# rrahn/libspm

Measured on AMD Instinct MI355X. Metric: Gbases/s scanned, Myers k<=3 |P|=100, higher is better.
Workload: dtype u32

## Files before the change

libspm_amd/csrc/filter.hpp:

```cpp
#pragma once

#include "brute.hpp"
#include "common.hpp"
#include "filter_shared.hpp"
#include "pack.hpp"
#include "hd.hpp"

namespace spm_hip
{

struct survivor
{
    uint32_t key;
    uint32_t t_lo, t_hi;
    uint32_t pad;
};
constexpr uint32_t kSurvInvalid = 0xFFFFFFFFu;

struct band_rec
{
    uint32_t slot;
    uint32_t val;
    uint32_t seg;
    uint32_t band;
};
constexpr uint32_t kBandInvalid = 0xFFFFFFFFu;
constexpr unsigned long long kBandEmpty = ~0ull;

constexpr uint32_t kChunkMax = 1024;
constexpr uint32_t kCandLdsSlot = 4;
constexpr uint32_t kCandRec = 8;

struct filter_params
{
    const uint8_t *text;
    uint64_t text_alloc;
    uint64_t lo, hi;
    uint32_t stride;
    uint32_t bitmap_words;
    uint32_t n_probes;
    uint32_t span_chunks;
    uint32_t span_unit;
    uint32_t dynamic;
    uint32_t key_len;
    uint32_t key_mask;
    uint32_t hash_variant;
    uint32_t lds_words;
    uint32_t chd_slot_mask;
    uint32_t chd_bucket_shift;
    uint32_t chd_disp_off;
    const uint32_t *bitmap;
    uint32_t span_budget;
    uint32_t pass;
    uint32_t anchor_c, anchor_cm;
    uint32_t n_pat, pat_c[kDensePatterns], pat_cm[kDensePatterns];
    uint32_t bucket_shift;
    const uint4 *buckets;
    survivor *surv;
    unsigned long long *counters;
    uint64_t surv_cap;
    uint64_t *ovf_spans;
    uint64_t ovf_cap;
};

__device__ __forceinline__ void wave_count_add(unsigned long long *counter, uint32_t v)
{
    for (int o = 32; o > 0; o >>= 1)
        v += __shfl_xor(v, o);
    if ((threadIdx.x & 63) == 0 && v)
        atomicAdd(counter, (unsigned long long)v);
}

__device__ __forceinline__ uint32_t *cand_chunk_of(const filter_params &P, const uint32_t *lds)
{
    const uint32_t wave = (uint32_t)__builtin_amdgcn_readfirstlane(threadIdx.x >> 6);
    return const_cast<uint32_t *>(lds) + P.lds_words + kCandLdsSlot + kCandRec * wave;
}

__device__ __forceinline__ void span_open(const filter_params &P, const uint32_t *lds, uint32_t lane, uint64_t begin)
{
    if (lane == 0) {
        uint32_t *ck = cand_chunk_of(P, lds);
        ck[4] = 0;
        ck[5] = 0;
        ck[6] = (uint32_t)begin;
        ck[7] = (uint32_t)(begin >> 32);
    }
}

__device__ __forceinline__ void span_give_up(const filter_params &P, uint32_t *ck, uint32_t lane)
{
    if (lane == 0) {
        ck[5] = 1;
        const unsigned long long i = atomicAdd(&P.counters[kCntSpansGaveUp], 1ull);
        if (i < P.ovf_cap) {
            P.ovf_spans[2 * i] = ((uint64_t)ck[7] << 32) | ck[6];
            P.ovf_spans[2 * i + 1] = (uint64_t)P.span_chunks * (uint64_t)P.span_unit;
        } else {
            atomicAdd(&P.counters[kCntVoid], 1ull);
        }
    }
    __builtin_amdgcn_fence(__ATOMIC_RELEASE, "wavefront");
    __builtin_amdgcn_wave_barrier();
}

__device__ __forceinline__ void surv_close(const filter_params &P, const uint32_t *ck, uint32_t lane)
{
    const uint32_t used = ck[2], size = ck[3];
    const uint64_t base = ((uint64_t)ck[1] << 32) | ck[0];
    for (uint32_t i = used + lane; i < size; i += 64)
        if (base + i < P.surv_cap) {
            survivor sv;
            sv.key = 0;
            sv.t_lo = 0;
            sv.t_hi = kSurvInvalid;
            sv.pad = 0;
            P.surv[base + i] = sv;
        }
}

__device__ __forceinline__ void emit_survivors(const filter_params &P, bool has, uint32_t key, uint64_t t, uint32_t lane,
                                               const uint32_t *lds)
{
    const uint64_t m = __ballot(has);
    if (m == 0)
        return;
    uint32_t *ck = cand_chunk_of(P, lds);
    const uint32_t n = __popcll(m);
    uint32_t used = (uint32_t)__builtin_amdgcn_readfirstlane(ck[2]);
    const uint32_t size = (uint32_t)__builtin_amdgcn_readfirstlane(ck[3]);
    const uint32_t cnt = (uint32_t)__builtin_amdgcn_readfirstlane(ck[4]) + n;
    if (cnt > P.span_budget) {
        span_give_up(P, ck, lane);
        return;
    }
    if (used + n > size) {
        surv_close(P, ck, lane);
        uint32_t next = size * 2 < kChunkMin ? kChunkMin : (size * 2 > kChunkMax ? kChunkMax : size * 2);
        next = next < n ? n : next;
        if (lane == 0) {
            const unsigned long long b = atomicAdd(&P.counters[kCntSurvSlots], (unsigned long long)next);
            ck[0] = (uint32_t)b;
            ck[1] = (uint32_t)(b >> 32);
            ck[2] = 0;
            ck[3] = next;
        }
        used = 0;
        __builtin_amdgcn_fence(__ATOMIC_RELEASE, "wavefront");
        __builtin_amdgcn_wave_barrier();
    }
    const uint64_t cbase = ((uint64_t)(uint32_t)__builtin_amdgcn_readfirstlane(ck[1]) << 32) |
                           (uint32_t)__builtin_amdgcn_readfirstlane(ck[0]);
    if (cbase + used + n > P.surv_cap) {
        span_give_up(P, ck, lane);
        return;
    }
    if (has) {
        survivor sv;
        sv.key = key;
        sv.t_lo = (uint32_t)t;
        sv.t_hi = (uint32_t)(t >> 32);
        sv.pad = P.pass;
        P.surv[cbase + used + __popcll(m & ((1ull << lane) - 1))] = sv;
    }
    if (lane == 0) {
        ck[2] = used + n;
        ck[4] = cnt;
    }
    __builtin_amdgcn_fence(__ATOMIC_RELEASE, "wavefront");
    __builtin_amdgcn_wave_barrier();
}

template <int S, int NWD, int HV, int SIG, bool PK, bool KM>
__device__ __forceinline__ void filter_words(const filter_params &P, const uint32_t (&w)[NWD],
                                             const uint32_t (&prev)[NWD], const uint32_t (&nv)[SIG != 4 ? NWD : 1],
                                             uint64_t gbase, uint32_t lane, const uint32_t *lds, uint32_t idx_mask)
{
    constexpr int NWIN = 16 / S;
    const uint32_t kmask = KM ? P.key_mask : 0xFFFFFFFFu;
    static_assert(NWD * NWIN <= 32, "one mask bit per window of a group");
    uint32_t pos_mask = 0;
    if constexpr (HV == 2) {
        const uint16_t *fp_tab = reinterpret_cast<const uint16_t *>(lds);
        const uint16_t *disp_tab = reinterpret_cast<const uint16_t *>(reinterpret_cast<const uint8_t *>(lds) + P.chd_disp_off);
        uint32_t xs[NWD * NWIN], ds[NWD * NWIN];
#pragma unroll
        for (int u = 0; u < NWD; ++u) {
#pragma unroll
            for (int i = 0; i < NWIN; ++i) {
                const int d = S * (i + 1);
                const uint32_t key = (d == 16 ? w[u] : alignbit(w[u], prev[u], (2 * d) & 31)) & kmask;
                const uint32_t x = chd_hash(key).x;
                xs[u * NWIN + i] = x;
                ds[u * NWIN + i] = disp_tab[x >> P.chd_bucket_shift];
            }
        }
#pragma unroll
        for (int u = 0; u < NWD; ++u) {
#pragma unroll
            for (int i = 0; i < NWIN; ++i) {
                const int d = S * (i + 1);
                const uint32_t key = (d == 16 ? w[u] : alignbit(w[u], prev[u], (2 * d) & 31)) & kmask;
                const uint32_t slot = ((xs[u * NWIN + i] >> 3) + ds[u * NWIN + i] * ((key | 1u) & 0xFFFFFFu)) &
                                      P.chd_slot_mask;
                ds[u * NWIN + i] = fp_tab[slot];
            }
        }
#pragma unroll
        for (int u = 0; u < NWD; ++u) {
#pragma unroll
            for (int i = 0; i < NWIN; ++i) {
                const int d = S * (i + 1);
                const uint32_t key = (d == 16 ? w[u] : alignbit(w[u], prev[u], (2 * d) & 31)) & kmask;
                const uint32_t miss = (ds[u * NWIN + i] ^ key ^ (key >> 16)) & 0xFFFFu;
                pos_mask |= (miss == 0 ? 1u : 0u) << (u * NWIN + i);
            }
        }
    } else {
#pragma unroll
        for (int u = 0; u < NWD; ++u) {
#pragma unroll
            for (int i = 0; i < NWIN; ++i) {
                const int d = S * (i + 1);
                const uint32_t key = (d == 16 ? w[u] : alignbit(w[u], prev[u], (2 * d) & 31)) & kmask;
                const uint32_t h = bloom_hash(key, 0) & idx_mask;
                const uint32_t word = lds[h >> 5];
                pos_mask |= __builtin_amdgcn_ubfe(word, h, 1) << (u * NWIN + i);
            }
        }
        for (uint32_t pr = 1; pr < P.n_probes; ++pr) {
            if (__ballot(pos_mask != 0) == 0)
                break;
            uint32_t keep = 0;
#pragma unroll
            for (int u = 0; u < NWD; ++u) {
#pragma unroll
                for (int i = 0; i < NWIN; ++i) {
                    if (pos_mask & (1u << (u * NWIN + i))) {
                        const int d = S * (i + 1);
                        const uint32_t key = (d == 16 ? w[u] : alignbit(w[u], prev[u], (2 * d) & 31)) & kmask;
                        const uint32_t h = bloom_hash(key, pr) & idx_mask;
                        const uint32_t word = lds[h >> 5];
                        keep |= __builtin_amdgcn_ubfe(word, h, 1) << (u * NWIN + i);
                    }
                }
            }
            pos_mask = keep;
        }
    }
    if constexpr (SIG != 4) {
        if (__ballot(pos_mask != 0) != 0) {
#pragma unroll
            for (int u = 0; u < NWD; ++u) {
#pragma unroll
                for (int i = 0; i < NWIN; ++i) {
                    const int d = S * (i + 1);
                    if (__builtin_amdgcn_ubfe(nv[u], d, P.key_len) != 0)
                        pos_mask &= ~(1u << (u * NWIN + i));
                }
            }
        }
    }
    while (__ballot(pos_mask != 0) != 0) {
        if (__builtin_amdgcn_readfirstlane(cand_chunk_of(P, lds)[5]) != 0)
            break;
        uint64_t t = 0;
        uint32_t key = 0;
        bool has = false;
        if (pos_mask != 0) {
            const int bit = __ffs(pos_mask) - 1;
            pos_mask &= pos_mask - 1;
            const int u = bit / NWIN, i = bit % NWIN;
            const int d = S * (i + 1);
            uint32_t wu = w[0], pu = prev[0];
#pragma unroll
            for (int q = 1; q < NWD; ++q)
                if (u == q) {
                    wu = w[q];
                    pu = prev[q];
                }
            key = (d == 16 ? wu : alignbit(wu, pu, (uint32_t)(2 * d) & 31u)) & kmask;
            const uint64_t wpos = PK ? gbase + (uint64_t)(u >> 2) * 4096 + (uint64_t)lane * 64 + (uint64_t)(u & 3) * 16
                                     : gbase + (uint64_t)u * 1024 + (uint64_t)lane * 16;
            const int64_t ts = (int64_t)wpos - 16 + d;
            if (ts >= (int64_t)P.lo && (uint64_t)ts + P.key_len <= P.hi) {
                t = (uint64_t)ts;
                has = true;
            }
        }
        emit_survivors(P, has, key, t, lane, lds);
    }
}



__device__ __forceinline__ uint32_t anchor_select(uint32_t w, uint32_t prev, uint32_t c, uint32_t cm)
{
    const uint32_t C0 = (c & 3u) * 0x55555555u, M0 = (cm & 3u) * 0x55555555u;
    const uint32_t C1 = (c >> 2) * 0x55555555u, M1 = (cm >> 2) * 0x55555555u;
    const uint32_t X = alignbit(w, prev, 2);
    const uint32_t Y = alignbit(w, prev, 4);
    uint32_t t = ((X ^ C0) & M0) | ((Y ^ C1) & M1);
    t |= t >> 1;
    return ~t & 0x55555555u;
}

template <int NWD>
__device__ __forceinline__ void filter_words_anchored(const filter_params &P, const uint32_t (&w)[NWD], const uint32_t (&prev)[NWD],
                                                      uint64_t gbase, uint32_t lane, const uint32_t *lds)
{
    static_assert(NWD % 2 == 0 || NWD == 1, "words are taken in pairs");
    const uint16_t *fp_tab = reinterpret_cast<const uint16_t *>(lds);
    const uint16_t *disp_tab = reinterpret_cast<const uint16_t *>(reinterpret_cast<const uint8_t *>(lds) + P.chd_disp_off);
#pragma unroll
    for (int j = 0; j < NWD; j += 2) {
        uint32_t todo = anchor_select(w[j], prev[j], P.anchor_c, P.anchor_cm);
        if (j + 1 < NWD)
            todo |= anchor_select(w[j + 1 < NWD ? j + 1 : j], prev[j + 1 < NWD ? j + 1 : j], P.anchor_c, P.anchor_cm) << 1;
        while (__ballot(todo != 0) != 0) {
            const bool act = todo != 0;
            const uint32_t b = act ? (uint32_t)__ffs(todo) - 1u : 0u;
            todo &= todo - 1;
            const uint32_t u = b & 1u, d = (b >> 1) + 1u;
            const uint32_t wu = (j + 1 < NWD && u) ? w[j + 1 < NWD ? j + 1 : j] : w[j];
            const uint32_t pu = (j + 1 < NWD && u) ? prev[j + 1 < NWD ? j + 1 : j] : prev[j];
            const uint32_t key = (uint32_t)((((uint64_t)wu << 32) | pu) >> (2 * d));
            const uint32_t x = chd_hash(key).x;
            const uint32_t dsp = disp_tab[x >> P.chd_bucket_shift];
            const uint32_t slot = ((x >> 3) + dsp * ((key | 1u) & 0xFFFFFFu)) & P.chd_slot_mask;
            const uint32_t f = fp_tab[slot];
            const bool hit = act && ((f ^ key ^ (key >> 16)) & 0xFFFFu) == 0;
            if (__ballot(hit) != 0) {
                if (__builtin_amdgcn_readfirstlane(cand_chunk_of(P, lds)[5]) != 0)
                    return;
                const uint64_t wpos = gbase + (uint64_t)(j + u) * 1024 + (uint64_t)lane * 16;
                const int64_t ts = (int64_t)wpos - 16 + (int64_t)d;
                const bool has = hit && ts >= (int64_t)P.lo && (uint64_t)ts + P.key_len <= P.hi;
                emit_survivors(P, has, key, has ? (uint64_t)ts : 0, lane, lds);
            }
        }
    }
}

template <int S, int UU, int HV, int SIG, bool KM, bool AN = false>
__device__ __forceinline__ void filter_group(const filter_params &P, const uint4 (&cur)[UU], uint64_t gbase,
                                             uint32_t &carry_in, uint32_t &carry_n, uint32_t lane,
                                             const uint32_t *lds, uint32_t idx_mask)
{
    uint32_t w[UU], prev[UU];
    uint32_t nv[SIG != 4 ? UU : 1];
#pragma unroll
    for (int u = 0; u < UU; ++u) {
        uint32_t nm = 0;
        w[u] = pack16_sig<SIG>(cur[u], nm);
        prev[u] = __builtin_amdgcn_update_dpp(0u, w[u], 0x138 , 0xF, 0xF, false);
        if (lane == 0)
            prev[u] = carry_in;
        carry_in = __builtin_amdgcn_readlane(w[u], 63);
        if (SIG != 4) {
            uint32_t np = __builtin_amdgcn_update_dpp(0u, nm, 0x138, 0xF, 0xF, false);
            if (lane == 0)
                np = carry_n;
            carry_n = __builtin_amdgcn_readlane(nm, 63);
            nv[u] = (nm << 16) | np;
        }
    }
    if constexpr (AN)
        filter_words_anchored<UU>(P, w, prev, gbase, lane, lds);
    else
        filter_words<S, UU, HV, SIG, false, KM>(P, w, prev, nv, gbase, lane, lds, idx_mask);
}

template <int S, int U, int HV, int SIG, bool KM, bool AN = false>
__global__ __launch_bounds__(((S == 1 && !KM && SIG == 4) || (S == 2 && U == 2)) ? 1024 : 512) void seed_filter_kernel(const filter_params P)
{
    extern __shared__ uint32_t lds[];
    for (uint32_t i = threadIdx.x; i < P.lds_words; i += blockDim.x)
        lds[i] = P.bitmap[i];
    if ((threadIdx.x & 63) == 0) {
        uint32_t *ck = lds + P.lds_words + kCandLdsSlot + kCandRec * (threadIdx.x >> 6);
        for (uint32_t i = 0; i < kCandRec; ++i)
            ck[i] = 0;
    }
    __syncthreads();

    const uint32_t lane = threadIdx.x & 63;
    const uint32_t waves_per_wg = blockDim.x >> 6;
    const uint64_t wave_id =
        (uint64_t)blockIdx.x * waves_per_wg + (uint32_t)__builtin_amdgcn_readfirstlane(threadIdx.x >> 6);
    const uint64_t n_waves = (uint64_t)gridDim.x * waves_per_wg;
    const uint32_t idx_mask = P.bitmap_words * 32 - 1;

    const uint64_t base0 = P.lo & ~1023ull;
    const uint64_t n_chunks = (P.hi - base0 + 1023) / 1024;
    const uint64_t n_whole = (P.hi - base0) / 1024;
    const uint64_t span = P.span_chunks;
    const uint64_t n_spans = (n_chunks + span - 1) / span;
    const uint8_t *lane_text = P.text + base0 + (uint64_t)lane * 16;

    const uint32_t wave_in_wg = (uint32_t)__builtin_amdgcn_readfirstlane(threadIdx.x >> 6);
    uint64_t sp = wave_id;
    for (;;) {
        if (P.dynamic == 1) {
            unsigned long long t = 0;
            if (lane == 0)
                t = atomicAdd(&P.counters[kCntSpanHead], 1ull);
            sp = ((unsigned long long)__builtin_amdgcn_readfirstlane((uint32_t)(t >> 32)) << 32) |
                 (uint32_t)__builtin_amdgcn_readfirstlane((uint32_t)t);
        } else if (P.dynamic == 2) {
            __syncthreads();
            if (threadIdx.x == 0) {
                const unsigned long long t = atomicAdd(&P.counters[kCntSpanHead], (unsigned long long)waves_per_wg);
                lds[P.lds_words] = (uint32_t)t;
                lds[P.lds_words + 1] = (uint32_t)(t >> 32);
            }
            __syncthreads();
            const uint64_t base = ((uint64_t)(uint32_t)__builtin_amdgcn_readfirstlane(lds[P.lds_words + 1]) << 32) |
                                  (uint32_t)__builtin_amdgcn_readfirstlane(lds[P.lds_words]);
            if (base >= n_spans)
                break;
            sp = base + wave_in_wg;
            if (sp >= n_spans)
                continue;
        }
        if (sp >= n_spans)
            break;
        const uint64_t c_begin = sp * span;
        const uint64_t c_end = c_begin + span < n_chunks ? c_begin + span : n_chunks;
        span_open(P, lds, lane, base0 + c_begin * 1024);
        uint32_t carry_in = 0, carry_n = 0;
        {
            const uint64_t cb = base0 + c_begin * 1024;
            if (cb >= 16 && lane == 0) {
                const uint4 before = load_text16(P.text, cb - 16, P.hi);
                carry_in = pack16_sig<SIG>(before, carry_n);
            }
            carry_in = __builtin_amdgcn_readfirstlane(carry_in);
            carry_n = __builtin_amdgcn_readfirstlane(carry_n);
        }
        uint64_t ch = c_begin;
        const uint64_t whole_end = c_end < n_whole ? c_end : n_whole;
        const uint64_t fast_end = c_begin + (whole_end > c_begin ? (whole_end - c_begin) / U * U : 0);
        if (ch < fast_end) {
            uint4 nxt[U];
#pragma unroll
            for (int u = 0; u < U; ++u)
                nxt[u] = load16_stream(lane_text + (ch + u) * 1024);
            for (; ch < fast_end; ch += U) {
                uint4 cur[U];
#pragma unroll
                for (int u = 0; u < U; ++u)
                    cur[u] = nxt[u];
                const bool more = ch + U < fast_end;
                const uint64_t pf = more ? ch + U : ch;
                const uint64_t ustride = more ? 1024 : 0;
#pragma unroll
                for (int u = 0; u < U; ++u)
                    nxt[u] = load16_stream(lane_text + pf * 1024 + (uint64_t)u * ustride);
                if constexpr (S <= 2)
                    __builtin_amdgcn_sched_barrier(0);
                filter_group<S, U, HV, SIG, KM, AN>(P, cur, base0 + ch * 1024, carry_in, carry_n, lane, lds, idx_mask);
            }
        }
        for (; ch < c_end; ++ch) {
            uint4 one[1];
            one[0] = load_text16(P.text, base0 + ch * 1024 + (uint64_t)lane * 16, P.hi);
            filter_group<S, 1, HV, SIG, KM, AN>(P, one, base0 + ch * 1024, carry_in, carry_n, lane, lds, idx_mask);
        }
        sp += n_waves;
    }
    surv_close(P, cand_chunk_of(P, lds), lane);
}

constexpr uint32_t kDenseQueueCap = 192;
constexpr int kDenseBatches = 3;

template <int NP>
__device__ __forceinline__ uint32_t dense_select(const filter_params &P, uint32_t w, uint32_t prev)
{
    const uint32_t X = alignbit(w, prev, 2);
    const uint32_t Y = alignbit(w, prev, 4);
    uint32_t sel = 0;
#pragma unroll
    for (int i = 0; i < NP; ++i) {
        const uint32_t C0 = (P.pat_c[i] & 3u) * 0x55555555u, M0 = (P.pat_cm[i] & 3u) * 0x55555555u;
        const uint32_t C1 = (P.pat_c[i] >> 2) * 0x55555555u, M1 = (P.pat_cm[i] >> 2) * 0x55555555u;
        uint32_t t = ((X ^ C0) & M0) | ((Y ^ C1) & M1);
        t |= t >> 1;
        sel |= ~t;
    }
    return sel & 0x55555555u;
}

struct dense_queue
{
    uint32_t key[kDenseQueueCap];
    uint32_t off[kDenseQueueCap];
};

__device__ __forceinline__ void dense_drain(const filter_params &P, dense_queue &Q, uint32_t &qn, bool all, uint64_t span_base,
                                            uint32_t lane, const uint32_t *lds)
{
    while (qn >= 64 || (all && qn != 0)) {
        const uint32_t nb_full = qn >> 6;
        uint32_t nb = all ? (qn + 63) >> 6 : nb_full;
        nb = nb > (uint32_t)kDenseBatches ? (uint32_t)kDenseBatches : nb;
        uint32_t key[kDenseBatches], off[kDenseBatches];
        uint4 bk[kDenseBatches];
        bool v[kDenseBatches];
#pragma unroll
        for (int b = 0; b < kDenseBatches; ++b) {
            const int32_t e = (int32_t)qn - 64 * b - 1 - (int32_t)lane;
            v[b] = (uint32_t)b < nb && e >= 0;
            key[b] = 0;
            off[b] = 0;
            bk[b] = make_uint4(0, 0, 0, 0);
            if (v[b]) {
                key[b] = Q.key[e];
                off[b] = Q.off[e];
                bk[b] = P.buckets[dense_bucket(key[b], P.bucket_shift)];
            }
        }
        qn = qn > 64 * nb ? qn - 64 * nb : 0;
#pragma unroll
        for (int b = 0; b < kDenseBatches; ++b) {
            if ((uint32_t)b >= nb)
                break;
            const uint32_t f2 = dense_fp(key[b]) * 0x00010001u;
            const uint32_t x0 = bk[b].x ^ f2, x1 = bk[b].y ^ f2, x2 = bk[b].z ^ f2, x3 = bk[b].w ^ f2;
            const uint32_t z = ((x0 - 0x00010001u) & ~x0) | ((x1 - 0x00010001u) & ~x1) | ((x2 - 0x00010001u) & ~x2) |
                               ((x3 - 0x00010001u) & ~x3);
            const bool hit = v[b] && ((z & 0x80008000u) != 0 || (bk[b].w >> 16) == kDenseAcceptAll);
            if (__ballot(hit) != 0) {
                if (__builtin_amdgcn_readfirstlane(cand_chunk_of(P, lds)[5]) == 0) {
                    const int64_t ts = (int64_t)span_base + (int64_t)off[b] - 16;
                    const bool has = hit && ts >= (int64_t)P.lo && (uint64_t)ts + P.key_len <= P.hi;
                    emit_survivors(P, has, key[b], has ? (uint64_t)ts : 0, lane, lds);
                }
            }
        }
    }
}

template <int UU, int NP, int S, bool KM>
__device__ __forceinline__ void dense_group(const filter_params &P, const uint4 (&cur)[UU], uint64_t gbase, uint64_t span_base,
                                            uint32_t &carry_in, uint32_t lane, const uint32_t *lds, dense_queue &Q, uint32_t &qn)
{
    static_assert(UU % 2 == 0 || UU == 1, "words are taken in pairs");
    uint32_t w[UU], prev[UU];
#pragma unroll
    for (int u = 0; u < UU; ++u) {
        w[u] = pack16(cur[u]);
        prev[u] = __builtin_amdgcn_update_dpp(0u, w[u], 0x138 , 0xF, 0xF, false);
        if (lane == 0)
            prev[u] = carry_in;
        carry_in = __builtin_amdgcn_readlane(w[u], 63);
    }
    const uint32_t goff = (uint32_t)(gbase - span_base) + lane * 16;
#pragma unroll
    for (int j = 0; j < UU; j += 2) {
        constexpr bool pair = UU > 1;
        const uint32_t w0 = w[j], p0 = prev[j], w1 = w[pair ? j + 1 : j], p1 = prev[pair ? j + 1 : j];
        const uint32_t kmask = KM ? P.key_mask : 0xFFFFFFFFu;
        static_assert(kDenseBloomBits == 20, "the word address below takes bits 5..19 of the index");
        uint32_t pm = 0;
        if constexpr (S == 0) {
            uint32_t todo = dense_select<NP>(P, w0, p0);
            if (pair)
                todo |= dense_select<NP>(P, w1, p1) << 1;
            while (todo != 0) {
                const uint32_t b = (uint32_t)__ffs(todo) - 1u;
                todo &= todo - 1;
                const bool odd = (b & 1u) != 0;
                const uint64_t both = ((uint64_t)(odd ? w1 : w0) << 32) | (odd ? p1 : p0);
                const uint32_t key = (uint32_t)(both >> ((b & ~1u) + 2u));
                const uint32_t h = key ^ (key >> 13);
                const uint32_t word = *reinterpret_cast<const uint32_t *>(reinterpret_cast<const uint8_t *>(lds) + ((h >> 3) & 0x1FFFCu));
                pm |= __builtin_amdgcn_ubfe(word, h, 1) << b;
            }
        } else {
#pragma unroll
            for (int u = 0; u < (pair ? 2 : 1); ++u) {
#pragma unroll
                for (int d = S; d <= 16; d += S) {
                    const uint32_t wu = u ? w1 : w0, pu = u ? p1 : p0;
                    const uint32_t key = (d == 16 ? wu : alignbit(wu, pu, (2 * d) & 31)) & kmask;
                    const uint32_t h = key ^ (key >> 13);
                    const uint32_t word = *reinterpret_cast<const uint32_t *>(reinterpret_cast<const uint8_t *>(lds) + ((h >> 3) & 0x1FFFCu));
                    pm |= __builtin_amdgcn_ubfe(word, h, 1) << (2 * (d - 1) + u);
                }
            }
        }
        while (__ballot(pm != 0) != 0) {
            const bool pos = pm != 0;
            const uint32_t b = pos ? (uint32_t)__ffs(pm) - 1u : 0u;
            pm &= pm - 1;
            const bool odd = (b & 1u) != 0;
            const uint64_t both = ((uint64_t)(odd ? w1 : w0) << 32) | (odd ? p1 : p0);
            const uint32_t key = (uint32_t)(both >> ((b & ~1u) + 2u)) & kmask;
            const uint64_t mm = __ballot(pos);
            if (pos) {
                const uint32_t q = qn + __popcll(mm & ((1ull << lane) - 1));
                Q.key[q] = key;
                Q.off[q] = goff + (uint32_t)j * 1024u + (odd ? 1024u : 0u) + (b >> 1) + 1u;
            }
            qn += __popcll(mm);
            __builtin_amdgcn_fence(__ATOMIC_RELEASE, "wavefront");
            __builtin_amdgcn_wave_barrier();
            if (qn > kDenseQueueCap - 64)
                dense_drain(P, Q, qn, false, span_base, lane, lds);
        }
    }
}

template <int U, int NP, int S = 0, bool KM = false>
__global__ __launch_bounds__(1024) void seed_filter_dense_kernel(const filter_params P)
{
    extern __shared__ uint32_t lds[];
    for (uint32_t i = threadIdx.x; i < P.lds_words; i += blockDim.x)
        lds[i] = P.bitmap[i];
    if ((threadIdx.x & 63) == 0) {
        uint32_t *ck = lds + P.lds_words + kCandLdsSlot + kCandRec * (threadIdx.x >> 6);
        for (uint32_t i = 0; i < kCandRec; ++i)
            ck[i] = 0;
    }
    __syncthreads();

    const uint32_t lane = threadIdx.x & 63;
    const uint32_t waves_per_wg = blockDim.x >> 6;
    const uint32_t wave_in_wg = (uint32_t)__builtin_amdgcn_readfirstlane(threadIdx.x >> 6);
    const uint64_t wave_id = (uint64_t)blockIdx.x * waves_per_wg + wave_in_wg;
    const uint64_t n_waves = (uint64_t)gridDim.x * waves_per_wg;
    dense_queue &Q = *reinterpret_cast<dense_queue *>(lds + P.lds_words + kCandLdsSlot + kCandRec * 16 +
                                                      (sizeof(dense_queue) / 4) * wave_in_wg);
    uint32_t qn = 0;

    const uint64_t base0 = P.lo & ~1023ull;
    const uint64_t n_chunks = (P.hi - base0 + 1023) / 1024;
    const uint64_t n_whole = (P.hi - base0) / 1024;
    const uint64_t span = P.span_chunks;
    const uint64_t n_spans = (n_chunks + span - 1) / span;
    const uint8_t *lane_text = P.text + base0 + (uint64_t)lane * 16;

    uint64_t sp = wave_id;
    for (;;) {
        if (P.dynamic == 1) {
            unsigned long long t = 0;
            if (lane == 0)
                t = atomicAdd(&P.counters[kCntSpanHead], 1ull);
            sp = ((unsigned long long)__builtin_amdgcn_readfirstlane((uint32_t)(t >> 32)) << 32) |
                 (uint32_t)__builtin_amdgcn_readfirstlane((uint32_t)t);
        } else if (P.dynamic == 2) {
            __syncthreads();
            if (threadIdx.x == 0) {
                const unsigned long long t = atomicAdd(&P.counters[kCntSpanHead], (unsigned long long)waves_per_wg);
                lds[P.lds_words] = (uint32_t)t;
                lds[P.lds_words + 1] = (uint32_t)(t >> 32);
            }
            __syncthreads();
            const uint64_t base = ((uint64_t)(uint32_t)__builtin_amdgcn_readfirstlane(lds[P.lds_words + 1]) << 32) |
                                  (uint32_t)__builtin_amdgcn_readfirstlane(lds[P.lds_words]);
            if (base >= n_spans)
                break;
            sp = base + wave_in_wg;
            if (sp >= n_spans)
                continue;
        }
        if (sp >= n_spans)
            break;
        const uint64_t c_begin = sp * span;
        const uint64_t c_end = c_begin + span < n_chunks ? c_begin + span : n_chunks;
        const uint64_t span_base = base0 + c_begin * 1024;
        span_open(P, lds, lane, span_base);
        uint32_t carry_in = 0;
        {
            uint32_t nm = 0;
            if (span_base >= 16 && lane == 0)
                carry_in = pack16_sig<4>(load_text16(P.text, span_base - 16, P.hi), nm);
            carry_in = __builtin_amdgcn_readfirstlane(carry_in);
        }
        uint64_t ch = c_begin;
        const uint64_t whole_end = c_end < n_whole ? c_end : n_whole;
        const uint64_t fast_end = c_begin + (whole_end > c_begin ? (whole_end - c_begin) / U * U : 0);
        if (ch < fast_end) {
            uint4 nxt[U];
#pragma unroll
            for (int u = 0; u < U; ++u)
                nxt[u] = load16_stream(lane_text + (ch + u) * 1024);
            for (; ch < fast_end; ch += U) {
                uint4 cur[U];
#pragma unroll
                for (int u = 0; u < U; ++u)
                    cur[u] = nxt[u];
                const bool more = ch + U < fast_end;
                const uint64_t pf = more ? ch + U : ch;
                const uint64_t ustride = more ? 1024 : 0;
#pragma unroll
                for (int u = 0; u < U; ++u)
                    nxt[u] = load16_stream(lane_text + pf * 1024 + (uint64_t)u * ustride);
                __builtin_amdgcn_sched_barrier(0);
                dense_group<U, NP, S, KM>(P, cur, base0 + ch * 1024, span_base, carry_in, lane, lds, Q, qn);
            }
        }
        for (; ch < c_end; ++ch) {
            uint4 one[1];
            one[0] = load_text16(P.text, base0 + ch * 1024 + (uint64_t)lane * 16, P.hi);
            dense_group<1, NP, S, KM>(P, one, base0 + ch * 1024, span_base, carry_in, lane, lds, Q, qn);
        }
        dense_drain(P, Q, qn, true, span_base, lane, lds);
        sp += n_waves;
    }
    surv_close(P, cand_chunk_of(P, lds), lane);
}

template <int S, int U2, int HV, bool KM>
__global__ __launch_bounds__(1024) void seed_filter_packed_kernel(const filter_params P, const uint4 *__restrict__ shadow)
{
    extern __shared__ uint32_t lds[];
    for (uint32_t i = threadIdx.x; i < P.lds_words; i += blockDim.x)
        lds[i] = P.bitmap[i];
    if ((threadIdx.x & 63) == 0) {
        uint32_t *ck = lds + P.lds_words + kCandLdsSlot + kCandRec * (threadIdx.x >> 6);
        for (uint32_t i = 0; i < kCandRec; ++i)
            ck[i] = 0;
    }
    __syncthreads();

    constexpr int NWD = 4 * U2;
    const uint32_t lane = threadIdx.x & 63;
    const uint32_t waves_per_wg = blockDim.x >> 6;
    const uint32_t wave_in_wg = (uint32_t)__builtin_amdgcn_readfirstlane(threadIdx.x >> 6);
    const uint64_t wave_id = (uint64_t)blockIdx.x * waves_per_wg + wave_in_wg;
    const uint64_t n_waves = (uint64_t)gridDim.x * waves_per_wg;
    const uint32_t idx_mask = P.bitmap_words * 32 - 1;

    const uint64_t base0 = P.lo & ~4095ull;
    const uint64_t n_chunks = (P.hi - base0 + 4095) / 4096;
    const uint64_t span = P.span_chunks;
    const uint64_t n_spans = (n_chunks + span - 1) / span;
    const uint4 *lane_src = shadow + (base0 / 64) + lane;

    uint64_t sp = wave_id;
    for (;;) {
        if (P.dynamic == 1) {
            unsigned long long t = 0;
            if (lane == 0)
                t = atomicAdd(&P.counters[kCntSpanHead], 1ull);
            sp = ((unsigned long long)__builtin_amdgcn_readfirstlane((uint32_t)(t >> 32)) << 32) |
                 (uint32_t)__builtin_amdgcn_readfirstlane((uint32_t)t);
        } else if (P.dynamic == 2) {
            __syncthreads();
            if (threadIdx.x == 0) {
                const unsigned long long t = atomicAdd(&P.counters[kCntSpanHead], (unsigned long long)waves_per_wg);
                lds[P.lds_words] = (uint32_t)t;
                lds[P.lds_words + 1] = (uint32_t)(t >> 32);
            }
            __syncthreads();
            const uint64_t base = ((uint64_t)(uint32_t)__builtin_amdgcn_readfirstlane(lds[P.lds_words + 1]) << 32) |
                                  (uint32_t)__builtin_amdgcn_readfirstlane(lds[P.lds_words]);
            if (base >= n_spans)
                break;
            sp = base + wave_in_wg;
            if (sp >= n_spans)
                continue;
        }
        if (sp >= n_spans)
            break;
        const uint64_t c_begin = sp * span;
        const uint64_t c_end = c_begin + span < n_chunks ? c_begin + span : n_chunks;
        const uint64_t fast_end = c_begin + (c_end - c_begin + U2 - 1) / U2 * U2;
        span_open(P, lds, lane, base0 + c_begin * 4096);
        uint32_t carry_in = 0;
        {
            const uint64_t first_word = (base0 + c_begin * 4096) / 16;
            if (first_word > 0 && lane == 0)
                carry_in = reinterpret_cast<const uint32_t *>(shadow)[first_word - 1];
            carry_in = __builtin_amdgcn_readfirstlane(carry_in);
        }
        uint4 nxt[U2];
#pragma unroll
        for (int u = 0; u < U2; ++u)
            nxt[u] = load16_stream(reinterpret_cast<const uint8_t *>(lane_src + (c_begin + u) * 64));
        for (uint64_t ch = c_begin; ch < fast_end; ch += U2) {
            uint4 cur[U2];
#pragma unroll
            for (int u = 0; u < U2; ++u)
                cur[u] = nxt[u];
            const bool more = ch + U2 < fast_end;
            const uint64_t pf = more ? ch + U2 : ch;
            const uint64_t ustride = more ? 64 : 0;
#pragma unroll
            for (int u = 0; u < U2; ++u)
                nxt[u] = load16_stream(reinterpret_cast<const uint8_t *>(lane_src + pf * 64 + (uint64_t)u * ustride));
            __builtin_amdgcn_sched_barrier(0);
            uint32_t w[NWD], prev[NWD];
            const uint32_t nv[1] = {0};
#pragma unroll
            for (int u = 0; u < U2; ++u) {
                w[4 * u + 0] = cur[u].x;
                w[4 * u + 1] = cur[u].y;
                w[4 * u + 2] = cur[u].z;
                w[4 * u + 3] = cur[u].w;
                uint32_t p0 = __builtin_amdgcn_update_dpp(0u, cur[u].w, 0x138 , 0xF, 0xF, false);
                if (lane == 0)
                    p0 = carry_in;
                carry_in = __builtin_amdgcn_readlane(cur[u].w, 63);
                prev[4 * u + 0] = p0;
                prev[4 * u + 1] = cur[u].x;
                prev[4 * u + 2] = cur[u].y;
                prev[4 * u + 3] = cur[u].z;
            }
            filter_words<S, NWD, HV, 4, true, KM>(P, w, prev, nv, base0 + ch * 4096, lane, lds, idx_mask);
        }
        sp += n_waves;
    }
    surv_close(P, cand_chunk_of(P, lds), lane);
}

struct verify_params
{
    const uint8_t *text;
    uint64_t text_alloc;
    uint64_t ctx_begin;
    uint64_t scan_begin;
    uint64_t scan_end;
    uint64_t pos_offset;
    const band_rec *bands;
    const unsigned long long *counters;
    uint32_t band_counter;
    uint32_t preselected;
    uint64_t band_cap;
    ulonglong2 *band_tab;
    uint32_t table_mask, band_bits;
    uint32_t runs;
    const uint8_t *surplus;
    uint32_t Bw;
    uint32_t overlap;
    uint32_t max_m;
    const uint32_t *peq32;
    uint32_t sigma;
    uint32_t nw_table;
    uint32_t max_k;
    const int32_t *m;
    const int32_t *k;
    uint32_t report_begin;
    uint32_t max_span;
    uint32_t wave_text;
    unsigned long long *seen;
    uint32_t seen_mask;
    spm_hit *hits;
    unsigned long long *hit_counter;
    uint64_t hit_cap;
    unsigned long long *overflow;
    const uint64_t *seg_offsets;
    uint64_t n_segments;
    const uint32_t *seg_owned;
};

struct resolve_params
{
    const survivor *surv;
    unsigned long long *counters;
    uint64_t surv_cap;
    const pass_entry *passes;
    const uint4 *entries;
    uint32_t key_len;
    uint32_t flank_check;
    uint32_t pieces_check;
    const uint8_t *text;
    uint64_t text_alloc;
    const uint8_t *needle_ranks;
    const uint32_t *needle_offsets;
    const uint16_t *seed_q;
    const int32_t *m, *k;
    uint64_t hay_begin, hay_end;
    const uint64_t *seg_offsets;
    uint64_t n_segments;
    uint32_t Bw, overlap, max_m;
    uint32_t band_bits;
    ulonglong2 *band_tab;
    uint32_t table_mask;
    band_rec *bands;
    uint64_t band_cap;
    const uint32_t *needle_pk;
    const uint32_t *pk_offsets;
    uint32_t exact_hits;
    uint32_t report_begin;
    uint64_t scan_begin, scan_end;
    uint64_t pos_offset;
    const uint32_t *seg_owned;
    unsigned long long *seen;
    uint32_t seen_mask;
    spm_hit *hits;
    unsigned long long *hit_counter, *overflow;
    uint64_t hit_cap;
    uint32_t *table_poison;
};

__device__ __forceinline__ unsigned long long band_value(unsigned long long stored, bool counting)
{
    return counting ? (unsigned long long)(uint32_t)(stored + 1ull) : ~stored;
}
__device__ __forceinline__ void band_release(ulonglong2 *tab, uint32_t slot)
{
    tab[slot] = make_ulonglong2(kBandEmpty, ~0ull);
}

__device__ __forceinline__ uint4 load_bytes16(const uint8_t *p)
{
    uint4 v;
    __builtin_memcpy(&v, p, 16);
    return v;
}

__device__ __forceinline__ uint4 load_bytes16_guarded(const uint8_t *base, uint64_t idx, uint64_t limit)
{
    if (idx + 16 <= limit)
        return load_bytes16(base + idx);
    uint32_t w[4] = {0xFFFFFFFFu, 0xFFFFFFFFu, 0xFFFFFFFFu, 0xFFFFFFFFu};
    for (int b = 0; b < 16; ++b)
        if (idx + b < limit)
            w[b >> 2] = (w[b >> 2] & ~(0xFFu << (8 * (b & 3)))) | ((uint32_t)base[idx + b] << (8 * (b & 3)));
    return make_uint4(w[0], w[1], w[2], w[3]);
}

__device__ __forceinline__ uint32_t diff16(const uint4 a, const uint4 b, uint32_t n)
{
    const uint32_t d[4] = {a.x ^ b.x, a.y ^ b.y, a.z ^ b.z, a.w ^ b.w};
    uint32_t r = 0;
#pragma unroll
    for (uint32_t i = 0; i < 4; ++i) {
        const uint32_t have = n > 4 * i ? n - 4 * i : 0;
        const uint32_t mask = have >= 4 ? 0xFFFFFFFFu : (have == 0 ? 0u : (1u << (8 * have)) - 1);
        r |= d[i] & mask;
    }
    return r;
}

__device__ __forceinline__ bool seed_intact(const resolve_params &P, uint64_t t, uint32_t val, uint32_t r, uint32_t q_whole,
                                            int64_t hay_b, int64_t hay_e)
{
    if (!P.needle_ranks)
        return true;
    const uint32_t pat = val >> 11, x = val & 0x7FF;
    struct
    {
        uint32_t q;
    } sp{q_whole ? q_whole : P.seed_q[pat]};
    const uint32_t o = x - r;
    const int64_t ts = (int64_t)t - (int64_t)r;
    if (ts < hay_b || ts + (int64_t)sp.q > hay_e)
        return false;
    const uint8_t *nd = P.needle_ranks + P.needle_offsets[pat] + o;
    for (uint32_t i = 0; i < sp.q; i += 16) {
        const uint32_t n = sp.q - i < 16 ? sp.q - i : 16;
        if (diff16(load_bytes16_guarded(P.text, (uint64_t)ts + i, P.text_alloc), load_bytes16(nd + i), n))
            return false;
    }
    return true;
}

constexpr uint32_t kPieceRoundsShift = 21, kPieceMissingShift = 28;

__device__ __forceinline__ bool pieces_apply(const resolve_params &P, uint64_t t, uint32_t val, uint32_t m, uint32_t k, int64_t hay_b,
                                             int64_t hay_e)
{
    if (!P.pieces_check || k == 0 || k > 7 || m < 32)
        return false;
    const int64_t d = (int64_t)t - (int64_t)(val & 0x7FF);
    return d - (int64_t)k >= hay_b && d + (int64_t)(m + k) <= hay_e;
}

__device__ __forceinline__ uint32_t pieces_visit(const resolve_params &P, uint64_t t, uint32_t val, uint32_t &rng, uint32_t m, uint32_t k)
{
    const uint32_t pat = val >> 11, x = val & 0x7FF;
    const uint32_t n_rounds = m >> 4;
    uint32_t done = (rng >> kPieceRoundsShift) & 0x7F, missing = (rng >> kPieceMissingShift) & 7;
    const bool ascending = 2 * x >= m;
    const uint32_t todo = n_rounds - done < 2 ? n_rounds - done : 2;
    const uint32_t r_lo = ascending ? done : n_rounds - done - todo;
    const uint32_t *pk = P.needle_pk + P.pk_offsets[pat] + r_lo;
    const uint32_t nw0 = pk[0], nw1 = todo == 2 ? pk[1] : 0;
    const uint64_t w0 = (uint64_t)((int64_t)t - (int64_t)x + (int64_t)(16 * r_lo) - (int64_t)k);
    const uint32_t c0 = pack16(load_bytes16_guarded(P.text, w0, P.text_alloc));
    const uint32_t c1 = pack16(load_bytes16_guarded(P.text, w0 + 16, P.text_alloc));
    const uint32_t c2 = todo == 2 ? pack16(load_bytes16_guarded(P.text, w0 + 32, P.text_alloc)) : 0;
#pragma unroll
    for (uint32_t rr = 0; rr < 2; ++rr) {
        if (rr < todo) {
            const uint32_t two = rr ? nw1 : nw0;
            const uint64_t win = rr ? ((uint64_t)c1 | ((uint64_t)c2 << 32)) : ((uint64_t)c0 | ((uint64_t)c1 << 32));
#pragma unroll
            for (uint32_t j = 0; j < 2; ++j) {
                const uint32_t piece = (two >> (16 * j)) & 0xFFFFu;
                bool found = false;
                for (uint32_t sh = 0; sh <= 2 * k; ++sh)
                    found = found || (((uint32_t)(win >> (2 * (8 * j + sh))) & 0xFFFFu) == piece);
                missing += found ? 0u : 1u;
            }
        }
    }
    if (missing > k)
        return 0;
    done += todo;
    if (done >= n_rounds)
        return 2;
    rng = (rng & ~((0x7Fu << kPieceRoundsShift) | (7u << kPieceMissingShift))) | (done << kPieceRoundsShift) |
          (missing << kPieceMissingShift);
    return 1;
}

struct text64
{
    uint64_t lo, hi;
    bool ok;
};

__device__ __forceinline__ uint32_t syms16(const text64 &W, uint32_t first)
{
    if (first >= 32)
        return (uint32_t)(W.hi >> (2 * (first - 32)));
    return (uint32_t)(W.lo >> (2 * first)) | (first ? (uint32_t)(W.hi << (2 * (32 - first)) ) : 0u);
}

__device__ __forceinline__ bool seed_sig_ok(const text64 &W, uint32_t sig, uint32_t r, uint32_t n, uint32_t H)
{
    if (n == 0)
        return true;
// ... 1093 lines not shown
```

Before: 6190.

## Overlap table staging and span prefetch with work draws in seed filter kernel

Bitmap staging into LDS is now done with 16-byte batched loads, and the helper is shared by all filter kernels. The main seed filter kernel issues the span atomic draw and the first text loads before staging the table. Inside the span loop it draws the next span ahead of time, so the loads for the next span's first group are issued during the last group of the current one. The main cost targeted is exposed latency at kernel start and at span boundaries, paid for with more complex control flow, extra registers, and a double-buffered LDS slot for the dynamic=2 handoff.

```diff
diff --git a/libspm_amd/csrc/filter.hpp b/libspm_amd/csrc/filter.hpp
--- a/libspm_amd/csrc/filter.hpp
+++ b/libspm_amd/csrc/filter.hpp
@@ -171,6 +171,42 @@
     __builtin_amdgcn_wave_barrier();
 }
 
+template <int B>
+__device__ __forceinline__ void stage_batches(const uint4 *src, uint4 *dst, uint32_t &i, uint32_t n16)
+{
+    const uint32_t bd = blockDim.x;
+    for (; i + (uint32_t)(B - 1) * bd < n16; i += (uint32_t)B * bd) {
+        uint4 v[B];
+#pragma unroll
+        for (int b = 0; b < B; ++b)
+            v[b] = src[i + (uint32_t)b * bd];
+#pragma unroll
+        for (int b = 0; b < B; ++b)
+            dst[i + (uint32_t)b * bd] = v[b];
+    }
+}
+
+__device__ __forceinline__ void stage_table(const filter_params &P, uint32_t *lds)
+{
+    const uint32_t n16 = (reinterpret_cast<uintptr_t>(P.bitmap) & 15u) == 0 ? P.lds_words >> 2 : 0u;
+    {
+        const uint4 *src = reinterpret_cast<const uint4 *>(P.bitmap);
+        uint4 *dst = reinterpret_cast<uint4 *>(lds);
+        uint32_t i = threadIdx.x;
+        stage_batches<8>(src, dst, i, n16);
+        stage_batches<4>(src, dst, i, n16);
+        stage_batches<2>(src, dst, i, n16);
+        stage_batches<1>(src, dst, i, n16);
+    }
+    for (uint32_t i = 4 * n16 + threadIdx.x; i < P.lds_words; i += blockDim.x)
+        lds[i] = P.bitmap[i];
+    if ((threadIdx.x & 63) == 0) {
+        uint32_t *ck = lds + P.lds_words + kCandLdsSlot + kCandRec * (threadIdx.x >> 6);
+        for (uint32_t i = 0; i < kCandRec; ++i)
+            ck[i] = 0;
+    }
+}
+
 template <int S, int NWD, int HV, int SIG, bool PK, bool KM>
 __device__ __forceinline__ void filter_words(const filter_params &P, const uint32_t (&w)[NWD],
                                              const uint32_t (&prev)[NWD], const uint32_t (&nv)[SIG != 4 ? NWD : 1],
@@ -343,26 +379,24 @@
 }
 
 template <int S, int UU, int HV, int SIG, bool KM, bool AN = false>
-__device__ __forceinline__ void filter_group(const filter_params &P, const uint4 (&cur)[UU], uint64_t gbase,
-                                             uint32_t &carry_in, uint32_t &carry_n, uint32_t lane,
-                                             const uint32_t *lds, uint32_t idx_mask)
-{
-    uint32_t w[UU], prev[UU];
+__device__ __forceinline__ void filter_packed(const filter_params &P, const uint32_t (&w)[UU], const uint32_t (&nm)[UU],
+                                              uint64_t gbase, uint32_t &carry_in, uint32_t &carry_n, uint32_t lane,
+                                              const uint32_t *lds, uint32_t idx_mask)
+{
+    uint32_t prev[UU];
     uint32_t nv[SIG != 4 ? UU : 1];
 #pragma unroll
     for (int u = 0; u < UU; ++u) {
-        uint32_t nm = 0;
-        w[u] = pack16_sig<SIG>(cur[u], nm);
         prev[u] = __builtin_amdgcn_update_dpp(0u, w[u], 0x138 , 0xF, 0xF, false);
         if (lane == 0)
             prev[u] = carry_in;
         carry_in = __builtin_amdgcn_readlane(w[u], 63);
         if (SIG != 4) {
-            uint32_t np = __builtin_amdgcn_update_dpp(0u, nm, 0x138, 0xF, 0xF, false);
+            uint32_t np = __builtin_amdgcn_update_dpp(0u, nm[u], 0x138, 0xF, 0xF, false);
             if (lane == 0)
                 np = carry_n;
-            carry_n = __builtin_amdgcn_readlane(nm, 63);
-            nv[u] = (nm << 16) | np;
+            carry_n = __builtin_amdgcn_readlane(nm[u], 63);
+            nv[u] = (nm[u] << 16) | np;
         }
     }
     if constexpr (AN)
@@ -371,23 +405,26 @@
         filter_words<S, UU, HV, SIG, false, KM>(P, w, prev, nv, gbase, lane, lds, idx_mask);
 }
 
+template <int S, int UU, int HV, int SIG, bool KM, bool AN = false>
+__device__ __forceinline__ void filter_group(const filter_params &P, const uint4 (&cur)[UU], uint64_t gbase,
+                                             uint32_t &carry_in, uint32_t &carry_n, uint32_t lane,
+                                             const uint32_t *lds, uint32_t idx_mask)
+{
+    uint32_t w[UU], nm[UU];
+#pragma unroll
+    for (int u = 0; u < UU; ++u)
+        w[u] = pack16_sig<SIG>(cur[u], nm[u]);
+    filter_packed<S, UU, HV, SIG, KM, AN>(P, w, nm, gbase, carry_in, carry_n, lane, lds, idx_mask);
+}
+
 template <int S, int U, int HV, int SIG, bool KM, bool AN = false>
 __global__ __launch_bounds__(((S == 1 && !KM && SIG == 4) || (S == 2 && U == 2)) ? 1024 : 512) void seed_filter_kernel(const filter_params P)
 {
     extern __shared__ uint32_t lds[];
-    for (uint32_t i = threadIdx.x; i < P.lds_words; i += blockDim.x)
-        lds[i] = P.bitmap[i];
-    if ((threadIdx.x & 63) == 0) {
-        uint32_t *ck = lds + P.lds_words + kCandLdsSlot + kCandRec * (threadIdx.x >> 6);
-        for (uint32_t i = 0; i < kCandRec; ++i)
-            ck[i] = 0;
-    }
-    __syncthreads();
-
     const uint32_t lane = threadIdx.x & 63;
     const uint32_t waves_per_wg = blockDim.x >> 6;
-    const uint64_t wave_id =
-        (uint64_t)blockIdx.x * waves_per_wg + (uint32_t)__builtin_amdgcn_readfirstlane(threadIdx.x >> 6);
+    const uint32_t wave_in_wg = (uint32_t)__builtin_amdgcn_readfirstlane(threadIdx.x >> 6);
+    const uint64_t wave_id = (uint64_t)blockIdx.x * waves_per_wg + wave_in_wg;
     const uint64_t n_waves = (uint64_t)gridDim.x * waves_per_wg;
     const uint32_t idx_mask = P.bitmap_words * 32 - 1;
 
@@ -398,76 +435,135 @@
     const uint64_t n_spans = (n_chunks + span - 1) / span;
     const uint8_t *lane_text = P.text + base0 + (uint64_t)lane * 16;
 
-    const uint32_t wave_in_wg = (uint32_t)__builtin_amdgcn_readfirstlane(threadIdx.x >> 6);
-    uint64_t sp = wave_id;
-    for (;;) {
+    unsigned long long tk = 0;
+    const bool drawer = P.dynamic == 1 ? lane == 0 : threadIdx.x == 0;
+    uint32_t opaque0 = 0;
+    asm volatile("" : "+v"(opaque0));
+    unsigned long long *head = P.counters + kCntSpanHead + opaque0;
+    auto draw = [&]() {
+        if (P.dynamic != 0 && drawer)
+            tk = atomicAdd(head, P.dynamic == 1 ? 1ull : (unsigned long long)waves_per_wg);
+    };
+    uint32_t round = 0;
+    bool wg_done = false;
+    auto take = [&](uint64_t after) -> uint64_t {
+        uint64_t next;
         if (P.dynamic == 1) {
-            unsigned long long t = 0;
-            if (lane == 0)
-                t = atomicAdd(&P.counters[kCntSpanHead], 1ull);
-            sp = ((unsigned long long)__builtin_amdgcn_readfirstlane((uint32_t)(t >> 32)) << 32) |
-                 (uint32_t)__builtin_amdgcn_readfirstlane((uint32_t)t);
+            next = ((unsigned long long)__builtin_amdgcn_readfirstlane((uint32_t)(tk >> 32)) << 32) |
+                   (uint32_t)__builtin_amdgcn_readfirstlane((uint32_t)tk);
+            wg_done = next >= n_spans;
         } else if (P.dynamic == 2) {
+            uint32_t *slot = lds + P.lds_words + 2 * (round & 1);
+            if (threadIdx.x == 0) {
+                slot[0] = (uint32_t)tk;
+                slot[1] = (uint32_t)(tk >> 32);
+            }
             __syncthreads();
-            if (threadIdx.x == 0) {
-                const unsigned long long t = atomicAdd(&P.counters[kCntSpanHead], (unsigned long long)waves_per_wg);
-                lds[P.lds_words] = (uint32_t)t;
-                lds[P.lds_words + 1] = (uint32_t)(t >> 32);
-            }
-            __syncthreads();
-            const uint64_t base = ((uint64_t)(uint32_t)__builtin_amdgcn_readfirstlane(lds[P.lds_words + 1]) << 32) |
-                                  (uint32_t)__builtin_amdgcn_readfirstlane(lds[P.lds_words]);
-            if (base >= n_spans)
-                break;
-            sp = base + wave_in_wg;
-            if (sp >= n_spans)
-                continue;
-        }
-        if (sp >= n_spans)
-            break;
-        const uint64_t c_begin = sp * span;
-        const uint64_t c_end = c_begin + span < n_chunks ? c_begin + span : n_chunks;
-        span_open(P, lds, lane, base0 + c_begin * 1024);
-        uint32_t carry_in = 0, carry_n = 0;
-        {
-            const uint64_t cb = base0 + c_begin * 1024;
-            if (cb >= 16 && lane == 0) {
-                const uint4 before = load_text16(P.text, cb - 16, P.hi);
-                carry_in = pack16_sig<SIG>(before, carry_n);
-            }
-            carry_in = __builtin_amdgcn_readfirstlane(carry_in);
-            carry_n = __builtin_amdgcn_readfirstlane(carry_n);
-        }
+            const uint64_t base = ((uint64_t)(uint32_t)__builtin_amdgcn_readfirstlane(slot[1]) << 32) |
+                                  (uint32_t)__builtin_amdgcn_readfirstlane(slot[0]);
+            wg_done = base >= n_spans;
+            next = base + wave_in_wg;
+        } else {
+            next = after + n_waves;
+            wg_done = next >= n_spans;
+        }
+        ++round;
+        return next;
+    };
+    auto first_group_whole = [&](uint64_t s) { return s < n_spans && s * span + U <= n_whole; };
+
+    uint4 nxt[U];
+    uint4 cw = make_uint4(0, 0, 0, 0);
+    bool primed = false;
+    uint64_t sp;
+    draw();
+    if (P.dynamic == 2) {
+        stage_table(P, lds);
+        sp = take(0);
+    } else {
+        sp = P.dynamic == 1 ? take(0) : wave_id;
+        wg_done = sp >= n_spans;
+        if (first_group_whole(sp)) {
+            const uint64_t c0 = sp * span;
+            const uint64_t cb = base0 + c0 * 1024;
+            cw = *reinterpret_cast<const uint4 *>(P.text + (cb >= 16 ? cb - 16 : cb));
+#pragma unroll
+            for (int u = 0; u < U; ++u)
+                nxt[u] = load16_stream(lane_text + (c0 + u) * 1024);
+            primed = true;
+        }
+        stage_table(P, lds);
+        __syncthreads();
+    }
+
+    while (!wg_done) {
+        const bool idle = sp >= n_spans;
+        const uint64_t c_begin = idle ? 0 : sp * span;
+        const uint64_t c_end = idle ? 0 : (c_begin + span < n_chunks ? c_begin + span : n_chunks);
+        const uint64_t cb = base0 + c_begin * 1024;
+        if (!idle)
+            span_open(P, lds, lane, cb);
         uint64_t ch = c_begin;
         const uint64_t whole_end = c_end < n_whole ? c_end : n_whole;
-        const uint64_t fast_end = c_begin + (whole_end > c_begin ? (whole_end - c_begin) / U * U : 0);
-        if (ch < fast_end) {
-            uint4 nxt[U];
-#pragma unroll
-            for (int u = 0; u < U; ++u)
-                nxt[u] = load16_stream(lane_text + (ch + u) * 1024);
-            for (; ch < fast_end; ch += U) {
-                uint4 cur[U];
+        const uint64_t n_groups = whole_end > c_begin ? (whole_end - c_begin) / U : 0;
+        uint32_t carry_in = 0, carry_n = 0;
+        if (primed) {
+            if (cb >= 16)
+                carry_in = pack16_sig<SIG>(cw, carry_n);
+        } else if (!idle) {
+            if (n_groups != 0) {
 #pragma unroll
                 for (int u = 0; u < U; ++u)
-                    cur[u] = nxt[u];
-                const bool more = ch + U < fast_end;
-                const uint64_t pf = more ? ch + U : ch;
-                const uint64_t ustride = more ? 1024 : 0;
-#pragma unroll
-                for (int u = 0; u < U; ++u)
-                    nxt[u] = load16_stream(lane_text + pf * 1024 + (uint64_t)u * ustride);
-                if constexpr (S <= 2)
-                    __builtin_amdgcn_sched_barrier(0);
-                filter_group<S, U, HV, SIG, KM, AN>(P, cur, base0 + ch * 1024, carry_in, carry_n, lane, lds, idx_mask);
-            }
+                    nxt[u] = load16_stream(lane_text + (ch + u) * 1024);
+            }
+            if (cb >= 16)
+                carry_in = pack16_sig<SIG>(load_text16(P.text, cb - 16, P.hi), carry_n);
+            asm volatile("" : "+v"(carry_in));
+        }
+        carry_in = __builtin_amdgcn_readfirstlane(carry_in);
+        carry_n = __builtin_amdgcn_readfirstlane(carry_n);
+        primed = false;
+        uint64_t sp_next = 0;
+        for (uint64_t g = 0;; ++g) {
+            const bool last = g + 1 >= n_groups;
+            if (g + 2 == n_groups)
+                draw();
+            if (last) {
+                if (n_groups < 2) {
+                    draw();
+                    tk = ((unsigned long long)__builtin_amdgcn_readfirstlane((uint32_t)(tk >> 32)) << 32) |
+                         (uint32_t)__builtin_amdgcn_readfirstlane((uint32_t)tk);
+                }
+                sp_next = take(sp);
+            }
+            if (n_groups == 0)
+                break;
+            const bool ahead = last && first_group_whole(sp_next);
+            const uint64_t pf = !last ? ch + U : (ahead ? sp_next * span : ch);
+            const uint64_t ustride = (!last || ahead) ? 1024 : 0;
+            if (ahead) {
+                const uint64_t nb = base0 + pf * 1024;
+                cw = *reinterpret_cast<const uint4 *>(P.text + nb - 16);
+                primed = true;
+            }
+            uint32_t w[U], nm[U];
+#pragma unroll
+            for (int u = 0; u < U; ++u) {
+                w[u] = pack16_sig<SIG>(nxt[u], nm[u]);
+                nxt[u] = load16_stream(lane_text + pf * 1024 + (uint64_t)u * ustride);
+            }
+            __builtin_amdgcn_sched_barrier(0);
+            filter_packed<S, U, HV, SIG, KM, AN>(P, w, nm, base0 + ch * 1024, carry_in, carry_n, lane, lds, idx_mask);
+            ch += U;
+            if (last)
+                break;
         }
         for (; ch < c_end; ++ch) {
             uint4 one[1];
             one[0] = load_text16(P.text, base0 + ch * 1024 + (uint64_t)lane * 16, P.hi);
             filter_group<S, 1, HV, SIG, KM, AN>(P, one, base0 + ch * 1024, carry_in, carry_n, lane, lds, idx_mask);
         }
-        sp += n_waves;
+        sp = sp_next;
     }
     surv_close(P, cand_chunk_of(P, lds), lane);
 }
@@ -617,13 +713,7 @@
 __global__ __launch_bounds__(1024) void seed_filter_dense_kernel(const filter_params P)
 {
     extern __shared__ uint32_t lds[];
-    for (uint32_t i = threadIdx.x; i < P.lds_words; i += blockDim.x)
-        lds[i] = P.bitmap[i];
-    if ((threadIdx.x & 63) == 0) {
-        uint32_t *ck = lds + P.lds_words + kCandLdsSlot + kCandRec * (threadIdx.x >> 6);
-        for (uint32_t i = 0; i < kCandRec; ++i)
-            ck[i] = 0;
-    }
+    stage_table(P, lds);
     __syncthreads();
 
     const uint32_t lane = threadIdx.x & 63;
@@ -717,13 +807,7 @@
 __global__ __launch_bounds__(1024) void seed_filter_packed_kernel(const filter_params P, const uint4 *__restrict__ shadow)
 {
     extern __shared__ uint32_t lds[];
-    for (uint32_t i = threadIdx.x; i < P.lds_words; i += blockDim.x)
-        lds[i] = P.bitmap[i];
-    if ((threadIdx.x & 63) == 0) {
-        uint32_t *ck = lds + P.lds_words + kCandLdsSlot + kCandRec * (threadIdx.x >> 6);
-        for (uint32_t i = 0; i < kCandRec; ++i)
-            ck[i] = 0;
-    }
+    stage_table(P, lds);
     __syncthreads();
 
     constexpr int NWD = 4 * U2;
```

After: 6125. 1.0% lower.
